# olegiy/manuscript-ocr

Measured on AMD Instinct MI355X. Metric: manuscript pages/sec end-to-end (EAST+TRBA) at 1/2/4/8 MI355X; CER vs CPU ref, higher is better.
Workload: dtype f32 (bf16x3 split operands on the 1x1 / Winograd-domain GEMMs, f32 accumulate)

## Files before the change

### include/msocr.h

```cpp
#ifndef MSOCR_H
#define MSOCR_H
#include <stdint.h>

#ifdef __cplusplus
extern "C" {
#endif

#define MSOCR_F32 0
#define MSOCR_BF16 1

#define MSOCR_OK 0
#define MSOCR_E_ARG (-1)
#define MSOCR_E_LAUNCH (-2)
#define MSOCR_E_NOGPU (-3)

#define MSOCR_CONV_RELU 1u
#define MSOCR_CONV_RESIDUAL 2u
#define MSOCR_CONV_POOL2 4u

typedef struct msocr_conv_desc {
  int32_t dtype;
  int32_t N, H, W, Cin;
  int64_t in_sN, in_sH, in_sW;
  int32_t KH, KW, stride_h, stride_w, pad_h, pad_w;
  int32_t Ho, Wo, Cout;
  int64_t out_ld;
  int64_t res_ld;
  uint32_t flags;
} msocr_conv_desc;

int msocr_conv2d(const msocr_conv_desc* d, const void* in, const void* weight, const float* bias,
                 const void* residual, void* out, void* stream);

#define MSOCR_WINO_2X2 0
#define MSOCR_WINO_4X2 1
#define MSOCR_WINO_4X4 2
int64_t msocr_winograd_workspace_bytes(const msocr_conv_desc* d, int form);
int msocr_winograd_weights_host(int form, const float* w_khwc_host, int Cout, int Cin, float* u_out_host);
int msocr_conv3x3_winograd(const msocr_conv_desc* d, int form, int split, const void* in, const void* u, const float* bias,
                           const void* residual, void* out, void* workspace, void* stream);
int msocr_winograd_input_transform(const msocr_conv_desc* d, int form, const void* in, void* workspace, void* stream);
int msocr_winograd_gemm(const msocr_conv_desc* d, int form, int split, const void* u, void* workspace, void* stream);
int msocr_winograd_output_transform(const msocr_conv_desc* d, int form, const void* workspace, const float* bias, const void* residual,
                                    void* out, void* stream);

int msocr_split_bf16x3_host(const float* w_host, int64_t n, uint16_t* planes_out_host);
int msocr_split_bf16x3_ktile_host(const float* w_host, int64_t nbatch, int64_t rows, int64_t k, uint16_t* planes_out_host);
int msocr_conv1x1_split(const msocr_conv_desc* d, const void* in, const void* weight_planes, const float* bias,
                        const void* residual, void* out, void* stream);
int msocr_conv2d_split(const msocr_conv_desc* d, const void* in, const void* weight_planes, const float* bias,
                       const void* residual, void* out, void* stream);

int64_t msocr_winograd_fused64_workspace_bytes(const msocr_conv_desc* d);
int msocr_conv3x3_winograd_fused64(const msocr_conv_desc* d, int split, const void* in, const void* u, const float* bias,
                                   const void* residual, void* out, void* workspace, void* stream);
int msocr_winograd_fused64_gemm_output(const msocr_conv_desc* d, int split, const void* u, const void* workspace, const float* bias,
                                       const void* residual, void* out, void* stream);

int msocr_normalize_u8(const uint8_t* src, int N, int H, int W, int pad_t, int pad_l, int Hp, int Wp, int cpad,
                       int mode, int dtype, void* out, void* stream);

int msocr_resize_linear_u8(const uint8_t* src, int N, int sh, int sw, uint8_t* dst, int dh, int dw, void* stream);

int msocr_maxpool2d(const void* in, int N, int H, int W, int C, int64_t in_ld, int k, int s, int p, int dtype,
                    void* out, int Ho, int Wo, int64_t out_ld, void* stream);

int msocr_upsample2x_bilinear(const void* in, int N, int H, int W, int C, int64_t in_ld, int dtype, void* out,
// ... 187 lines not shown
```

### manuscript_ocr_amd/_native.py

```python
import ctypes
import os

import torch

_HERE = os.path.dirname(os.path.abspath(__file__))
LIB_PATH = os.path.join(_HERE, "libmsocr.so")

F32, BF16 = 0, 1
CONV_RELU, CONV_RESIDUAL, CONV_POOL2 = 1, 2, 4
WINO_2X2, WINO_4X2, WINO_4X4 = 0, 1, 2

c_i32, c_i64, c_u32 = ctypes.c_int32, ctypes.c_int64, ctypes.c_uint32
c_f32, c_f64, c_vp = ctypes.c_float, ctypes.c_double, ctypes.c_void_p


class ConvDesc(ctypes.Structure):
    _fields_ = [
        ("dtype", c_i32), ("N", c_i32), ("H", c_i32), ("W", c_i32), ("Cin", c_i32),
        ("in_sN", c_i64), ("in_sH", c_i64), ("in_sW", c_i64),
        ("KH", c_i32), ("KW", c_i32), ("stride_h", c_i32), ("stride_w", c_i32), ("pad_h", c_i32), ("pad_w", c_i32),
        ("Ho", c_i32), ("Wo", c_i32), ("Cout", c_i32),
        ("out_ld", c_i64), ("res_ld", c_i64), ("flags", c_u32),
    ]


class JpegInfo(ctypes.Structure):
    _fields_ = [("width", c_i32), ("height", c_i32), ("ncomp", c_i32), ("hs", c_i32 * 3), ("vs", c_i32 * 3),
                ("blocks_w", c_i32 * 3), ("blocks_h", c_i32 * 3), ("supported", c_i32), ("coef_off", c_i64 * 3),
                ("coef_total", c_i64), ("quant", (ctypes.c_uint16 * 64) * 3)]


class AttnWeights(ctypes.Structure):
    _fields_ = [(n, c_vp) for n in ("h2h_wt", "h2h_b", "score_w", "wih_ctx_t", "wih_tok", "whh_t", "b_gates", "gen_wt", "gen_b")]


class AttnSplitWeights(ctypes.Structure):
    _fields_ = [(n, c_vp) for n in ("h2h_p", "whh_p", "gen_p")]


_SIGS = {
    "msocr_conv2d": (c_i32, [ctypes.POINTER(ConvDesc), c_vp, c_vp, c_vp, c_vp, c_vp, c_vp]),
    "msocr_winograd_workspace_bytes": (c_i64, [ctypes.POINTER(ConvDesc), c_i32]),
    "msocr_winograd_weights_host": (c_i32, [c_i32, c_vp, c_i32, c_i32, c_vp]),
    "msocr_conv3x3_winograd": (c_i32, [ctypes.POINTER(ConvDesc), c_i32, c_i32, c_vp, c_vp, c_vp, c_vp, c_vp, c_vp, c_vp]),
    "msocr_winograd_input_transform": (c_i32, [ctypes.POINTER(ConvDesc), c_i32, c_vp, c_vp, c_vp]),
    "msocr_winograd_gemm": (c_i32, [ctypes.POINTER(ConvDesc), c_i32, c_i32, c_vp, c_vp, c_vp]),
    "msocr_winograd_output_transform": (c_i32, [ctypes.POINTER(ConvDesc), c_i32, c_vp, c_vp, c_vp, c_vp, c_vp]),
    "msocr_winograd_fused64_workspace_bytes": (c_i64, [ctypes.POINTER(ConvDesc)]),
    "msocr_conv3x3_winograd_fused64": (c_i32, [ctypes.POINTER(ConvDesc), c_i32, c_vp, c_vp, c_vp, c_vp, c_vp, c_vp, c_vp]),
    "msocr_winograd_fused64_gemm_output": (c_i32, [ctypes.POINTER(ConvDesc), c_i32, c_vp, c_vp, c_vp, c_vp, c_vp, c_vp]),
    "msocr_split_bf16x3_host": (c_i32, [c_vp, c_i64, c_vp]),
    "msocr_split_bf16x3_ktile_host": (c_i32, [c_vp, c_i64, c_i64, c_i64, c_vp]),
    "msocr_conv1x1_split": (c_i32, [ctypes.POINTER(ConvDesc), c_vp, c_vp, c_vp, c_vp, c_vp, c_vp]),
    "msocr_conv2d_split": (c_i32, [ctypes.POINTER(ConvDesc), c_vp, c_vp, c_vp, c_vp, c_vp, c_vp]),
    "msocr_normalize_u8": (c_i32, [c_vp, c_i32, c_i32, c_i32, c_i32, c_i32, c_i32, c_i32, c_i32, c_i32, c_i32, c_vp, c_vp]),
    "msocr_resize_linear_u8": (c_i32, [c_vp, c_i32, c_i32, c_i32, c_vp, c_i32, c_i32, c_vp]),
    "msocr_maxpool2d": (c_i32, [c_vp, c_i32, c_i32, c_i32, c_i32, c_i64, c_i32, c_i32, c_i32, c_i32, c_vp, c_i32, c_i32, c_i64, c_vp]),
    "msocr_upsample2x_bilinear": (c_i32, [c_vp, c_i32, c_i32, c_i32, c_i32, c_i64, c_i32, c_vp, c_i64, c_vp]),
    "msocr_east_head": (c_i32, [c_vp, c_i64, c_i64, c_i32, c_vp, c_vp, c_vp, c_vp, c_vp]),
    "msocr_east_decode": (c_i32, [c_vp, c_vp, c_i32, c_i32, c_i32, c_f32, c_f32, c_i32, c_vp, c_vp, c_i32, c_vp]),
    "msocr_lanms_workspace_bytes": (c_i64, [c_i32, c_i32]),
    "msocr_east_lanms": (c_i32, [c_vp, c_vp, c_i32, c_i32, c_f64, c_vp, c_vp, c_vp, c_vp]),
    "msocr_se_residual": (c_i32, [c_vp, c_vp, c_i32, c_i32, c_i32, c_i32, c_vp, c_vp, c_vp, c_vp, c_vp]),
    "msocr_mean_over_h": (c_i32, [c_vp, c_i32, c_i32, c_i32, c_i32, c_i32, c_vp, c_vp]),
    "msocr_bilstm_recurrent": (c_i32, [c_vp, c_vp, c_i32, c_i32, c_i32, c_vp, c_vp]),
    "msocr_bilstm_recurrent_split": (c_i32, [c_vp, c_vp, c_i32, c_i32, c_i32, c_vp, c_vp]),
    "msocr_attn_greedy": (c_i32, [c_vp, c_vp, ctypes.POINTER(AttnWeights), c_i32, c_i32, c_i32, c_i32, c_i32, c_i32, c_i32, c_i32,
                                  c_vp, c_vp, c_vp]),
    "msocr_attn_greedy_hoisted": (c_i32, [c_vp, c_vp, c_vp, ctypes.POINTER(AttnWeights), ctypes.POINTER(AttnSplitWeights), c_i32, c_i32,
                                          c_i32, c_i32, c_i32, c_i32, c_i32, c_i32, c_vp, c_vp, c_vp]),
# ... 105 lines not shown
```

### manuscript_ocr_amd/csrc/winograd.hip

```cpp
#include <hip/hip_runtime.h>
#include <stdint.h>

#include "conv_common.h"

template <int M> __device__ void wino_bt1(const f32x4 d[M + 2], f32x4 r[M + 2]);
template <int M> __device__ void wino_at1(const f32x4 m[M + 2], f32x4 y[M]);

template <> __device__ __forceinline__ void wino_bt1<2>(const f32x4 d[4], f32x4 r[4]) {
  r[0] = d[0] - d[2];
  r[1] = d[1] + d[2];
  r[2] = d[2] - d[1];
  r[3] = d[1] - d[3];
}
template <> __device__ __forceinline__ void wino_at1<2>(const f32x4 m[4], f32x4 y[2]) {
  y[0] = (m[0] + m[1]) + m[2];
  y[1] = (m[1] - m[2]) - m[3];
}

__device__ __forceinline__ void wino44_bt(const f32x4 d[6], f32x4 r[6]) {
  constexpr float k97_36 = 97.0f / 36.0f, k4_9 = 4.0f / 9.0f, k9_4 = 2.25f, k3_2 = 1.5f, k2_3 = 2.0f / 3.0f;
#pragma unroll
  for (int e = 0; e < 4; ++e) {
    r[0][e] = fmaf(-k97_36, d[2][e], d[0][e]) + d[4][e];
    r[5][e] = fmaf(-k97_36, d[3][e], d[1][e]) + d[5][e];
    const float e1 = fmaf(-k4_9, d[2][e], d[4][e]), o1 = fmaf(k3_2, d[3][e], -k2_3 * d[1][e]);
    const float e2 = fmaf(-k9_4, d[2][e], d[4][e]), o2 = fmaf(k2_3, d[3][e], -k3_2 * d[1][e]);
    r[1][e] = e1 + o1; r[2][e] = e1 - o1;
    r[3][e] = e2 + o2; r[4][e] = e2 - o2;
  }
}
__device__ __forceinline__ void wino44_at(const f32x4 m[6], f32x4 y[4]) {
  constexpr float k3_2 = 1.5f, k2_3 = 2.0f / 3.0f, k9_4 = 2.25f, k4_9 = 4.0f / 9.0f, k27_8 = 3.375f, k8_27 = 8.0f / 27.0f;
#pragma unroll
  for (int e = 0; e < 4; ++e) {
    const float p12 = m[1][e] + m[2][e], d12 = m[1][e] - m[2][e], p34 = m[3][e] + m[4][e], d34 = m[3][e] - m[4][e];
    y[0][e] = (m[0][e] + p12) + p34;
    y[1][e] = fmaf(k3_2, d12, k2_3 * d34);
    y[2][e] = fmaf(k9_4, p12, k4_9 * p34);
    y[3][e] = fmaf(k27_8, d12, k8_27 * d34) + m[5][e];
  }
}
template <> __device__ __forceinline__ void wino_bt1<4>(const f32x4 d[6], f32x4 r[6]) { wino44_bt(d, r); }
template <> __device__ __forceinline__ void wino_at1<4>(const f32x4 m[6], f32x4 y[4]) { wino44_at(m, y); }


struct WinoGeom {
  int N, H, W;
  int TH, TW;
  long Mt;
};

template <int MH, int MW>
__device__ __forceinline__ void wino_input_body(const float* in, long sN, long sH, long sW, int C, WinoGeom g, float* V) {
  constexpr int PH = MH + 2, PW = MW + 2;
  constexpr bool w_first = MH == 4;
  const int cch = C >> 2;
  const long gid = (long)blockIdx.x * 256 + threadIdx.x;
  const long t = gid / cch;
  const int c = (int)(gid - t * cch) << 2;
  if (t >= g.Mt) return;
  const int tw = (int)(t % g.TW);
  const long r = t / g.TW;
  const int th = (int)(r % g.TH);
  const int n = (int)(r / g.TH);
  const int h0 = MH * th - 1, w0 = MW * tw - 1;
  const float* base = in + (long)n * sN + c;
  f32x4 q[PH][PW];
#pragma unroll
  for (int i = 0; i < PH; ++i) {
    const int hi = h0 + i;
    const bool okh = (unsigned)hi < (unsigned)g.H;
    f32x4 d[PW];
#pragma unroll
    for (int j = 0; j < PW; ++j) {
      const int wi = w0 + j;
      const bool ok = okh && (unsigned)wi < (unsigned)g.W;
      const f32x4 v = *reinterpret_cast<const f32x4*>(ok ? base + (long)hi * sH + (long)wi * sW : base);
      d[j] = ok ? v : (f32x4){0.f, 0.f, 0.f, 0.f};
    }
    if constexpr (w_first) {
      wino_bt1<MW>(d, q[i]);
    } else {
#pragma unroll
      for (int j = 0; j < PW; ++j) q[i][j] = d[j];
    }
  }
  const long plane = g.Mt * (long)C;
  float* o = V + t * (long)C + c;
// ... 7 lines not shown
#pragma unroll
      for (int i = 0; i < PH; ++i) *reinterpret_cast<f32x4*>(o + (i * PW + j) * plane) = v[i];
    }
  } else {
#pragma unroll
    for (int i = 0; i < PH; ++i) {
      f32x4 row[PW], v[PW];
#pragma unroll
      for (int j = 0; j < PW; ++j) {
        f32x4 col[PH], hv[PH];
#pragma unroll
        for (int k = 0; k < PH; ++k) col[k] = q[k][j];
        wino_bt1<MH>(col, hv);
        row[j] = hv[i];
      }
      wino_bt1<MW>(row, v);
#pragma unroll
      for (int j = 0; j < PW; ++j) *reinterpret_cast<f32x4*>(o + (i * PW + j) * plane) = v[j];
    }
  }
}

template <int MH, int MW>
__device__ __forceinline__ void wino_output_body(const float* Mw, int Cout, WinoGeom g, const float* bias, const float* res, long res_ld,
                                                 int relu, float* out, long out_ld) {
  constexpr int PH = MH + 2, PW = MW + 2;
  const int cch = Cout >> 2;
  const long gid = (long)blockIdx.x * 256 + threadIdx.x;
  const long t = gid / cch;
  const int c = (int)(gid - t * cch) << 2;
  if (t >= g.Mt) return;
  const int tw = (int)(t % g.TW);
  const long r = t / g.TW;
  const int th = (int)(r % g.TH);
  const int n = (int)(r / g.TH);
  const long plane = g.Mt * (long)Cout;
  const float* mp = Mw + t * (long)Cout + c;
  f32x4 mt[PH][PW];
  if constexpr (MH == 2) {
#pragma unroll
    for (int i = 0; i < PH; ++i)
#pragma unroll
      for (int j = 0; j < PW; ++j) mt[i][j] = *reinterpret_cast<const f32x4*>(mp + (i * PW + j) * plane);
  }
  f32x4 s[MH][PW];
#pragma unroll
  for (int j = 0; j < PW; ++j) {
    f32x4 m[PH], y[MH];
#pragma unroll
    for (int i = 0; i < PH; ++i) m[i] = MH == 2 ? mt[i][j] : *reinterpret_cast<const f32x4*>(mp + (i * PW + j) * plane);
    wino_at1<MH>(m, y);
#pragma unroll
    for (int a = 0; a < MH; ++a) s[a][j] = y[a];
  }
  f32x4 b = {0.f, 0.f, 0.f, 0.f};
  if (bias) b = *reinterpret_cast<const f32x4*>(bias + c);
#pragma unroll
  for (int a = 0; a < MH; ++a) {
    const int ho = MH * th + a;
    if (ho >= g.H) continue;
    f32x4 y[MW];
    wino_at1<MW>(s[a], y);
#pragma unroll
    for (int j = 0; j < MW; ++j) {
      const int wo = MW * tw + j;
      if (wo >= g.W) continue;
      const long pix = ((long)n * g.H + ho) * g.W + wo;
      f32x4 v = y[j] + b;
      if (res) v += *reinterpret_cast<const f32x4*>(res + pix * res_ld + c);
      if (relu) {
        v[0] = fmaxf(v[0], 0.f); v[1] = fmaxf(v[1], 0.f); v[2] = fmaxf(v[2], 0.f); v[3] = fmaxf(v[3], 0.f);
      }
      *reinterpret_cast<f32x4*>(out + pix * out_ld + c) = v;
    }
  }
}

#define WINO_TRANSFORM_KERNELS(PREFIX, MH, MW)                                                                                    \
  __global__ __launch_bounds__(256) void PREFIX##_input_kernel(const float* __restrict__ in, long sN, long sH, long sW, int C,   \
                                                               WinoGeom g, float* __restrict__ V) {                            \
    wino_input_body<MH, MW>(in, sN, sH, sW, C, g, V);                                                                            \
  }                                                                                                                              \
  __global__ __launch_bounds__(256) void PREFIX##_output_kernel(const float* __restrict__ Mw, int Cout, WinoGeom g,              \
                                                                const float* __restrict__ bias, const float* __restrict__ res,  \
                                                                long res_ld, int relu, float* __restrict__ out, long out_ld) {  \
    wino_output_body<MH, MW>(Mw, Cout, g, bias, res, res_ld, relu, out, out_ld);                                                 \
  }
WINO_TRANSFORM_KERNELS(wino, 2, 2)
WINO_TRANSFORM_KERNELS(wino42, 4, 2)
WINO_TRANSFORM_KERNELS(wino44, 4, 4)
#undef WINO_TRANSFORM_KERNELS

static const int kWinoTile[3][2] = {{2, 2}, {4, 2}, {4, 4}};

static int wino_points(int form) { return (kWinoTile[form][0] + 2) * (kWinoTile[form][1] + 2); }

static bool wino_geom(const msocr_conv_desc* d, int form, WinoGeom* g) {
  if (form < MSOCR_WINO_2X2 || form > MSOCR_WINO_4X4 || !d || d->dtype != MSOCR_F32) return false;
  if (d->KH != 3 || d->KW != 3 || d->stride_h != 1 || d->stride_w != 1 || d->pad_h != 1 || d->pad_w != 1) return false;
  if (d->N <= 0 || d->H <= 0 || d->W <= 0 || d->Ho != d->H || d->Wo != d->W) return false;
  if (d->Cin <= 0 || d->Cin % 16 || d->Cout <= 0 || d->Cout % 32) return false;
  if ((long)d->N * ((d->H + 1) / 2) * ((d->W + 1) / 2) > 0x7fffffffL) return false;
  const int mh = kWinoTile[form][0], mw = kWinoTile[form][1];
  g->N = d->N; g->H = d->H; g->W = d->W;
  g->TH = (d->H + mh - 1) / mh; g->TW = (d->W + mw - 1) / mw;
  g->Mt = (long)d->N * g->TH * g->TW;
  return wino_points(form) * g->Mt * (long)(d->Cin > d->Cout ? d->Cin : d->Cout) <= 0x3fffffffffffL;
}

static bool wino_strides_ok(const msocr_conv_desc* d) { return !(d->in_sN % 4 || d->in_sH % 4 || d->in_sW % 4); }

static int wino_check(const msocr_conv_desc* d, int form, WinoGeom* g) {
  if (!wino_geom(d, form, g) || !wino_strides_ok(d) || d->out_ld % 4 || d->out_ld < d->Cout) return MSOCR_E_ARG;
  return MSOCR_OK;
}

static bool wino_gemm_ok(int form, int split) {
  if (split != 0 && split != 1) return false;
  return form == MSOCR_WINO_4X2 || (form == MSOCR_WINO_2X2 && !split) || (form == MSOCR_WINO_4X4 && split);
}

extern "C" int64_t msocr_winograd_workspace_bytes(const msocr_conv_desc* d, int form) {
  WinoGeom g;
  if (!wino_geom(d, form, &g)) return -1;
  return wino_points(form) * g.Mt * ((int64_t)d->Cin + d->Cout) * (int64_t)sizeof(float);
}

static int wino_launch_input(const msocr_conv_desc* d, int form, const WinoGeom& g, const void* in, void* workspace, void* stream) {
// ... 37 lines not shown
  if (bias && ((uintptr_t)bias & 15)) return MSOCR_E_ARG;
  const long nb_out = (g.Mt * (d->Cout / 4) + 255) / 256;
  if (nb_out > 0x7fffffffL) return MSOCR_E_ARG;
  const float* Mw = (const float*)workspace + wino_points(form) * g.Mt * (long)d->Cin;
  const float* rp = has_res ? (const float*)residual : nullptr;
  const int relu = (d->flags & MSOCR_CONV_RELU) ? 1 : 0;
  const dim3 grid((unsigned)nb_out), blk(256);
  hipStream_t st = (hipStream_t)stream;
  float* o = (float*)out;
  if (form == MSOCR_WINO_2X2) MSOCR_LAUNCH(wino_output_kernel, grid, blk, 0, st, Mw, d->Cout, g, bias, rp, (long)d->res_ld, relu, o, (long)d->out_ld);
  else if (form == MSOCR_WINO_4X2) MSOCR_LAUNCH(wino42_output_kernel, grid, blk, 0, st, Mw, d->Cout, g, bias, rp, (long)d->res_ld, relu, o, (long)d->out_ld);
  else MSOCR_LAUNCH(wino44_output_kernel, grid, blk, 0, st, Mw, d->Cout, g, bias, rp, (long)d->res_ld, relu, o, (long)d->out_ld);
  return hipGetLastError() == hipSuccess ? MSOCR_OK : MSOCR_E_LAUNCH;
}

extern "C" int msocr_conv3x3_winograd(const msocr_conv_desc* d, int form, int split, const void* in, const void* u, const float* bias,
                                      const void* residual, void* out, void* workspace, void* stream) {
  if (!u || !wino_gemm_ok(form, split)) return MSOCR_E_ARG;
  int rc = msocr_winograd_input_transform(d, form, in, workspace, stream);
  if (rc != MSOCR_OK) return rc;
  rc = msocr_winograd_gemm(d, form, split, u, workspace, stream);
  if (rc != MSOCR_OK) return rc;
  return msocr_winograd_output_transform(d, form, workspace, bias, residual, out, stream);
}

typedef unsigned int u32x4w __attribute__((ext_vector_type(4)));
#ifndef WINO_FUSED_PFD
#define WINO_FUSED_PFD 3
#endif

typedef __bf16 bf16x8w __attribute__((ext_vector_type(8)));
typedef unsigned int u32x2w __attribute__((ext_vector_type(2)));
template <bool POOL, bool SPLIT = false>
__global__ __launch_bounds__(256, 3) void wino42_fused64_kernel(const float* __restrict__ V, const void* __restrict__ Uv, int Cout,
                                                                 WinoGeom g, const float* __restrict__ bias,
                                                                 const float* __restrict__ res, long res_ld, int relu,
                                                                 float* __restrict__ out, long out_ld) {
  constexpr int K = 64, BM = 32, BN = 32, ROWB = K * 4;
  constexpr int ROWS = 128, PLANE = BM * ROWS;
  constexpr int STAGE_BYTES = SPLIT ? 6 * PLANE : (BM + BN) * ROWB;
  __shared__ __attribute__((aligned(16))) unsigned char smem[2][STAGE_BYTES];
  const int tid = threadIdx.x, lane = tid & 63, wave = tid >> 6;
  const int mi = wave >> 1, nj = wave & 1;
  const int r16 = lane & 15, kg = lane >> 4;
  const int nbn = Cout / BN;
  const long bid = xcd_tile<long>(blockIdx.x, gridDim.x);
// ... 370 lines not shown
    else
      MSOCR_LAUNCH((wino42_fused64_v2_kernel<false>), grid2, blk, 0, st, ws, up, d->Cout, g, bias, rp, (long)d->res_ld, relu, (float*)out, (long)d->out_ld);
    return hipGetLastError() == hipSuccess ? MSOCR_OK : MSOCR_E_LAUNCH;
  }
  if (d->flags & MSOCR_CONV_POOL2) {
    if (split) MSOCR_LAUNCH((wino42_fused64_kernel<true, true>), grid, blk, 0, st, ws, u, d->Cout, g, bias, (const float*)nullptr, 0L, relu, (float*)out, (long)d->out_ld);
    else MSOCR_LAUNCH((wino42_fused64_kernel<true, false>), grid, blk, 0, st, ws, u, d->Cout, g, bias, (const float*)nullptr, 0L, relu, (float*)out, (long)d->out_ld);
  } else {
    if (split) MSOCR_LAUNCH((wino42_fused64_kernel<false, true>), grid, blk, 0, st, ws, u, d->Cout, g, bias, rp, (long)d->res_ld, relu, (float*)out, (long)d->out_ld);
    else MSOCR_LAUNCH((wino42_fused64_kernel<false, false>), grid, blk, 0, st, ws, u, d->Cout, g, bias, rp, (long)d->res_ld, relu, (float*)out, (long)d->out_ld);
  }
  return hipGetLastError() == hipSuccess ? MSOCR_OK : MSOCR_E_LAUNCH;
}

extern "C" int msocr_conv3x3_winograd_fused64(const msocr_conv_desc* d, int split, const void* in, const void* u, const float* bias,
                                              const void* residual, void* out, void* workspace, void* stream) {
  WinoGeom g;
  if ((split != 0 && split != 1) || wino_fused64_check(d, &g) != MSOCR_OK || !u) return MSOCR_E_ARG;
  const int rc = wino_launch_input(d, MSOCR_WINO_4X2, g, in, workspace, stream);
  if (rc != MSOCR_OK) return rc;
  return msocr_winograd_fused64_gemm_output(d, split, u, workspace, bias, residual, out, stream);
}

extern "C" int msocr_winograd_weights_host(int form, const float* w_khwc, int Cout, int Cin, float* u_out) {
  if (form < MSOCR_WINO_2X2 || form > MSOCR_WINO_4X4 || !w_khwc || !u_out || Cout <= 0 || Cin <= 0) return MSOCR_E_ARG;
  static const double G4[4][3] = {{1.0, 0.0, 0.0}, {0.5, 0.5, 0.5}, {0.5, -0.5, 0.5}, {0.0, 0.0, 1.0}};
  static const double G6[6][3] = {{1.0, 0.0, 0.0},
                                  {8.0 / 65, 12.0 / 65, 18.0 / 65},     {8.0 / 65, -12.0 / 65, 18.0 / 65},
                                  {-81.0 / 130, -27.0 / 65, -18.0 / 65}, {-81.0 / 130, 27.0 / 65, -18.0 / 65},
                                  {0.0, 0.0, 1.0}};
  const int PH = kWinoTile[form][0] + 2, PW = kWinoTile[form][1] + 2;
  const double(*Gh)[3] = PH == 6 ? G6 : G4;
  const double(*Gw)[3] = PW == 6 ? G6 : G4;
  const long plane = (long)Cout * Cin;
  for (int co = 0; co < Cout; ++co) {
    const float* w = w_khwc + (long)co * 9 * Cin;
    for (int c = 0; c < Cin; ++c) {
      double gw[6][3];
      for (int xi = 0; xi < PH; ++xi)
        for (int kw = 0; kw < 3; ++kw)
          gw[xi][kw] = Gh[xi][0] * w[(0 * 3 + kw) * Cin + c] + Gh[xi][1] * w[(1 * 3 + kw) * Cin + c] + Gh[xi][2] * w[(2 * 3 + kw) * Cin + c];
      for (int xi = 0; xi < PH; ++xi)
        for (int nu = 0; nu < PW; ++nu)
          u_out[(xi * PW + nu) * plane + (long)co * Cin + c] =
              (float)(gw[xi][0] * Gw[nu][0] + gw[xi][1] * Gw[nu][1] + gw[xi][2] * Gw[nu][2]);
    }
  }
  return MSOCR_OK;
}
```

### manuscript_ocr_amd/ops.py

```python
import ctypes
import os
from typing import NamedTuple

import numpy as np
import torch

from . import _native as nat


PROFILE = None


def _prof_begin():
    if PROFILE is None:
        return None
    e0 = torch.cuda.Event(enable_timing=True)
    e0.record()
    return e0


def _prof_end(e0, kind, work, tag=None):
    if e0 is None or PROFILE is None:
        return
    e1 = torch.cuda.Event(enable_timing=True)
# ... 38 lines not shown
    if torch.cuda.is_current_stream_capturing():
        return torch.empty((nbytes,), dtype=torch.uint8, device=device)
    key = (device.index, torch.cuda.current_stream().cuda_stream)
    buf = _WINO_ARENA.get(key)
    if buf is None or buf.numel() < nbytes:
        buf = None
        _WINO_ARENA.pop(key, None)
        buf = torch.empty((nbytes,), dtype=torch.uint8, device=device)
        _WINO_ARENA[key] = buf
    return buf


WINOGRAD_TALL = int(os.environ.get("MSOCR_WINO_TALL", "1"))


def _tall_pays(H):
    return 24 * (-(-H // 4)) < 16 * (-(-H // 2))


WINOGRAD_SQUARE = int(os.environ.get("MSOCR_WINO_SQUARE", "1"))
WINOGRAD_SQUARE_MIN_CIN = int(os.environ.get("MSOCR_WINO_SQUARE_MIN_CIN", "512"))


def _square_pays(W):
    return 36 * (-(-W // 4)) < 24 * (-(-W // 2))


WINO_FORMS = {nat.WINO_2X2: ("winograd", 16, (2, 2)), nat.WINO_4X2: ("winograd42", 24, (4, 2)), nat.WINO_4X4: ("winograd44", 36, (4, 4))}


def _wino_weights(wh, form):
    Cout, _, _, Cin = wh.shape
    u = torch.empty((WINO_FORMS[form][1], Cout, Cin), dtype=torch.float32)
    nat.check(nat.lib().msocr_winograd_weights_host(form, wh.data_ptr(), Cout, Cin, u.data_ptr()), "winograd_weights_host")
    return u


WINOGRAD_FUSED64 = int(os.environ.get("MSOCR_WINO_FUSED64", "1"))


SPLIT_BF16X3 = int(os.environ.get("MSOCR_SPLIT", "1"))


def split_planes(t):
    th = t.detach().float().cpu().contiguous()
    planes = torch.empty((3,) + tuple(th.shape), dtype=torch.int16)
    nat.check(nat.lib().msocr_split_bf16x3_host(th.data_ptr(), th.numel(), planes.data_ptr()), "split_bf16x3_host")
    return planes.view(torch.bfloat16).to(t.device)


def split_planes_ktile(t, nbatch, rows):
    th = t.detach().float().cpu().contiguous()
    k = th.numel() // (nbatch * rows)
    assert k % 32 == 0 and nbatch * rows * k == th.numel()
    planes = torch.empty((3, nbatch, k // 32, rows, 32), dtype=torch.int16)
# ... 24 lines not shown
    return w


def attach_winograd(w, split=None, square=True):
    Cout, KH, KW, Cin = w.shape
    if (WINOGRAD_MIN_CIN and WINOGRAD_FUSED64 and WINOGRAD_TALL and w.dtype == torch.float32 and KH == 3 and KW == 3 and Cin == 64
            and Cin < WINOGRAD_MIN_CIN and Cout % 32 == 0):
        u42 = _wino_weights(w.detach().cpu().contiguous(), nat.WINO_4X2)
        w._msocr_wino42_fused = u42.to(w.device)
        if (SPLIT_BF16X3 if split is None else split) and (Cout % 64 == 0 or Cout >= 128):
            w._msocr_wino42_fused_split = split_planes(u42).to(w.device)
        return w
    if not (WINOGRAD_MIN_CIN and w.dtype == torch.float32 and KH == 3 and KW == 3 and Cin >= WINOGRAD_MIN_CIN and Cin % 16 == 0
            and Cout % 32 == 0):
        return w
    wh = w.detach().cpu().contiguous()
    w._msocr_wino = _wino_weights(wh, nat.WINO_2X2).to(w.device)
    u42 = _wino_weights(wh, nat.WINO_4X2)
    w._msocr_wino42 = u42.to(w.device)
    if (SPLIT_BF16X3 if split is None else split) and Cin % 32 == 0 and Cout % 64 == 0:
        w._msocr_wino42_split = split_planes_ktile(u42, 24, Cout).to(w.device)
        if WINOGRAD_SQUARE and square and Cin >= WINOGRAD_SQUARE_MIN_CIN:
            w._msocr_wino44_split = split_planes_ktile(_wino_weights(wh, nat.WINO_4X4), 36, Cout).to(w.device)
    return w


def _winograd(d, x, w, u, form, split, bias, residual, out, alg, fused=False, pool2=False):
    N, H, W, Cin = x.shape
    Cout = w.shape[0]
    stem, npts, (mh, mw) = WINO_FORMS[form]
    name = stem + ("_fused" if fused else "") + ("_split" if split else "")
    L = nat.lib()
    nbytes = L.msocr_winograd_fused64_workspace_bytes(ctypes.byref(d)) if fused else L.msocr_winograd_workspace_bytes(ctypes.byref(d), form)
    if nbytes < 0:
        raise nat.NativeError(f"{name}: unsupported shape {tuple(x.shape)} * {tuple(w.shape)} pool2={pool2}")
    parts = min(N, -(-nbytes // WINO_WS_LIMIT))
    per = -(-N // parts)
    ws = _wino_workspace(nbytes if parts == 1 else (nbytes // N) * per, x.device)
    bp = bias.data_ptr() if bias is not None else None
    what = f"msocr_conv3x3_{name} {tuple(x.shape)} * {tuple(w.shape)}"
    TH, TW = -(-H // mh), -(-W // mw)
    out_px = H * W // (4 if pool2 else 1)
    res_io = 2 if residual is not None else 1
    for n0 in range(0, N, per):
        n1 = min(N, n0 + per)
        d.N = n1 - n0
        xp, rp, op = x[n0:n1].data_ptr(), (residual[n0:n1].data_ptr() if residual is not None else None), out[n0:n1].data_ptr()
        if PROFILE is None:
            if fused:
                rc = L.msocr_conv3x3_winograd_fused64(ctypes.byref(d), int(split), xp, u.data_ptr(), bp, rp, op, ws.data_ptr(), _stream())
            else:
                rc = L.msocr_conv3x3_winograd(ctypes.byref(d), form, int(split), xp, u.data_ptr(), bp, rp, op, ws.data_ptr(), _stream())
            nat.check(rc, what)
            continue
        nn, mt = n1 - n0, (n1 - n0) * TH * TW
        e = _prof_begin()
        nat.check(L.msocr_winograd_input_transform(ctypes.byref(d), form, xp, ws.data_ptr(), _stream()), what)
        _prof_end(e, "wino_in", 4.0 * (nn * H * W * Cin + npts * mt * Cin), (mt, Cin))
        e = _prof_begin()
        if fused:
            rc = L.msocr_winograd_fused64_gemm_output(ctypes.byref(d), int(split), u.data_ptr(), ws.data_ptr(), bp, rp, op, _stream())
        else:
            rc = L.msocr_winograd_gemm(ctypes.byref(d), form, int(split), u.data_ptr(), ws.data_ptr(), _stream())
        nat.check(rc, what)
        io = x.element_size() * (nn * H * W * Cin + nn * out_px * Cout * res_io + Cout * 9 * Cin)
        _prof_end(e, "conv_gemm", (alg * nn / N, 2.0 * npts * mt * Cin * Cout, io), (nn * H * W, Cout, 9 * Cin, name))
        if not fused:
            e = _prof_begin()
            nat.check(L.msocr_winograd_output_transform(ctypes.byref(d), form, ws.data_ptr(), bp, rp, op, _stream()), what)
            _prof_end(e, "wino_out", 4.0 * (npts * mt * Cout + nn * H * W * Cout * res_io), (mt, Cout))
    d.N = N


def conv2d(x, w, bias, stride=(1, 1), pad=(0, 0), relu=False, residual=None, out=None, out_hw=None, alg_k=None, pool2=False):
    _need_cuda(x, w, bias, residual, out)
    N, H, W, Cin = x.shape
    Cout, KH, KW, Cw = w.shape
    assert Cw == Cin and w.is_contiguous() and w.dtype == x.dtype and x.stride(3) == 1
# ... 15 lines not shown
    d.dtype = _dt(x)
    d.N, d.H, d.W, d.Cin = N, H, W, Cin
    d.in_sN, d.in_sH, d.in_sW = x.stride(0), x.stride(1), x.stride(2)
    d.KH, d.KW, d.stride_h, d.stride_w, d.pad_h, d.pad_w = KH, KW, sh, sw, ph, pw
    d.Ho, d.Wo, d.Cout = Ho, Wo, Cout
    d.out_ld = _pixel_dense_ld(out)
    flags = (nat.CONV_RELU if relu else 0) | (nat.CONV_POOL2 if pool2 else 0)
    rp = None
    if residual is not None:
        assert residual.shape == out.shape and residual.dtype == x.dtype
        d.res_ld = _pixel_dense_ld(residual)
        flags |= nat.CONV_RESIDUAL
        rp = residual.data_ptr()
    d.flags = flags
    if bias is not None:
        assert bias.dtype == torch.float32 and bias.numel() == Cout and bias.is_contiguous()
    bp = bias.data_ptr() if bias is not None else None
    alg = 2.0 * N * Ho * Wo * Cout * (alg_k if alg_k else KH * KW * Cin)
    if fused:
        up = getattr(w, "_msocr_wino42_fused_split", None) if SPLIT_BF16X3 else None
        u = w._msocr_wino42_fused if up is None else up
        _winograd(d, x, w, u, nat.WINO_4X2, up is not None, bias, residual, out, alg, fused=True, pool2=pool2)
    elif use_wino:
        form, split = nat.WINO_2X2, False
        if WINOGRAD_TALL and _tall_pays(H) and getattr(w, "_msocr_wino42", None) is not None:
            form, u = nat.WINO_4X2, w._msocr_wino42
            up = getattr(w, "_msocr_wino42_split", None)
            if up is not None and SPLIT_BF16X3:
                u, split = up, True
            up44 = getattr(w, "_msocr_wino44_split", None)
            if up44 is not None and SPLIT_BF16X3 and WINOGRAD_SQUARE and _square_pays(W):
                form, u, split = nat.WINO_4X4, up44, True
        _winograd(d, x, w, u, form, split, bias, residual, out, alg)
    else:
        wp = getattr(w, "_msocr_split", None)
        if (wp is None and SPLIT_BF16X3 and not getattr(w, "_msocr_nosplit", False) and _split_eligible(w)
                and not torch.cuda.is_current_stream_capturing()):
            wp = w._msocr_split = split_planes_ktile(w, 1, Cout)
        split = wp is not None and SPLIT_BF16X3 and KH * KW * Cin >= SPLIT_MIN_K and all(v % 4 == 0 for v in x.stride()[:3])
        lean = (split and (KH, KW, sh, sw, ph, pw) == (1, 1, 1, 1, 0, 0) and (Ho, Wo) == (H, W)
                and (H == 1 or x.stride(1) == W * x.stride(2)) and (N == 1 or x.stride(0) == H * W * x.stride(2)))
        e = _prof_begin()
        if split:
            fn = nat.lib().msocr_conv1x1_split if lean else nat.lib().msocr_conv2d_split
            rc = fn(ctypes.byref(d), x.data_ptr(), wp.data_ptr(), bp, rp, out.data_ptr(), _stream())
            nat.check(rc, f"msocr_conv{'1x1' if lean else '2d'}_split {tuple(x.shape)} * {tuple(w.shape)}")
        else:
            rc = nat.lib().msocr_conv2d(ctypes.byref(d), x.data_ptr(), w.data_ptr(), bp, rp, out.data_ptr(), _stream())
            nat.check(rc, f"msocr_conv2d {tuple(x.shape)} * {tuple(w.shape)}")
        io = x.element_size() * (N * H * W * Cin + N * Ho * Wo * Cout * (2 if residual is not None else 1) + Cout * KH * KW * Cin)
        _prof_end(e, "conv_gemm", (alg, 2.0 * N * Ho * Wo * Cout * KH * KW * Cin, io),
                  (N * Ho * Wo, Cout, KH * KW * Cin, "direct_split" if split else "direct"))
    return out


def normalize_u8(imgs_u8, pad_t, pad_l, Hp, Wp, mode, dtype, cpad=4):
# ... 313 lines not shown
```

Before: 79.79.

## Add F(4x4) Winograd with F(4x1) column tail for widths of form 4k+1

For 3x3 convs whose width is 4k+1, the change splits tiles into a 4x4 Winograd main region plus a single-column 4x1 tail (18 transform points) instead of padding a whole extra 4x4 tile column. It adds combined input and output transform kernels, tail weight transforms, and two batched split-bf16 GEMMs, and updates the square-pays heuristic to account for the cheaper tail. The aim is to cut wasted GEMM work on padded columns, which may also make 4x4 eligible for more layers. In exchange it adds an extra GEMM launch and more workspace complexity.

```diff
diff --git a/include/msocr.h b/include/msocr.h
--- a/include/msocr.h
+++ b/include/msocr.h
@@ -43,6 +43,15 @@
 int msocr_winograd_gemm(const msocr_conv_desc* d, int form, int split, const void* u, void* workspace, void* stream);
 int msocr_winograd_output_transform(const msocr_conv_desc* d, int form, const void* workspace, const float* bias, const void* residual,
                                     void* out, void* stream);
+
+int64_t msocr_winograd_coltail_workspace_bytes(const msocr_conv_desc* d);
+int msocr_winograd_coltail_weights_host(const float* w_khwc_host, int Cout, int Cin, float* u_out_host);
+int msocr_conv3x3_winograd_coltail(const msocr_conv_desc* d, const void* in, const void* u44, const void* u41, const float* bias,
+                                   const void* residual, void* out, void* workspace, void* stream);
+int msocr_winograd_coltail_input_transform(const msocr_conv_desc* d, const void* in, void* workspace, void* stream);
+int msocr_winograd_coltail_gemm(const msocr_conv_desc* d, const void* u44, const void* u41, void* workspace, void* stream);
+int msocr_winograd_coltail_output_transform(const msocr_conv_desc* d, const void* workspace, const float* bias, const void* residual,
+                                            void* out, void* stream);
 
 int msocr_split_bf16x3_host(const float* w_host, int64_t n, uint16_t* planes_out_host);
 int msocr_split_bf16x3_ktile_host(const float* w_host, int64_t nbatch, int64_t rows, int64_t k, uint16_t* planes_out_host);
diff --git a/manuscript_ocr_amd/_native.py b/manuscript_ocr_amd/_native.py
--- a/manuscript_ocr_amd/_native.py
+++ b/manuscript_ocr_amd/_native.py
@@ -46,6 +46,12 @@
     "msocr_winograd_input_transform": (c_i32, [ctypes.POINTER(ConvDesc), c_i32, c_vp, c_vp, c_vp]),
     "msocr_winograd_gemm": (c_i32, [ctypes.POINTER(ConvDesc), c_i32, c_i32, c_vp, c_vp, c_vp]),
     "msocr_winograd_output_transform": (c_i32, [ctypes.POINTER(ConvDesc), c_i32, c_vp, c_vp, c_vp, c_vp, c_vp]),
+    "msocr_winograd_coltail_workspace_bytes": (c_i64, [ctypes.POINTER(ConvDesc)]),
+    "msocr_winograd_coltail_weights_host": (c_i32, [c_vp, c_i32, c_i32, c_vp]),
+    "msocr_conv3x3_winograd_coltail": (c_i32, [ctypes.POINTER(ConvDesc), c_vp, c_vp, c_vp, c_vp, c_vp, c_vp, c_vp, c_vp]),
+    "msocr_winograd_coltail_input_transform": (c_i32, [ctypes.POINTER(ConvDesc), c_vp, c_vp, c_vp]),
+    "msocr_winograd_coltail_gemm": (c_i32, [ctypes.POINTER(ConvDesc), c_vp, c_vp, c_vp, c_vp]),
+    "msocr_winograd_coltail_output_transform": (c_i32, [ctypes.POINTER(ConvDesc), c_vp, c_vp, c_vp, c_vp, c_vp]),
     "msocr_winograd_fused64_workspace_bytes": (c_i64, [ctypes.POINTER(ConvDesc)]),
     "msocr_conv3x3_winograd_fused64": (c_i32, [ctypes.POINTER(ConvDesc), c_i32, c_vp, c_vp, c_vp, c_vp, c_vp, c_vp, c_vp]),
     "msocr_winograd_fused64_gemm_output": (c_i32, [ctypes.POINTER(ConvDesc), c_i32, c_vp, c_vp, c_vp, c_vp, c_vp, c_vp]),
diff --git a/manuscript_ocr_amd/csrc/winograd.hip b/manuscript_ocr_amd/csrc/winograd.hip
--- a/manuscript_ocr_amd/csrc/winograd.hip
+++ b/manuscript_ocr_amd/csrc/winograd.hip
@@ -43,27 +43,29 @@
 template <> __device__ __forceinline__ void wino_bt1<4>(const f32x4 d[6], f32x4 r[6]) { wino44_bt(d, r); }
 template <> __device__ __forceinline__ void wino_at1<4>(const f32x4 m[6], f32x4 y[4]) { wino44_at(m, y); }
 
+template <> __device__ __forceinline__ void wino_bt1<1>(const f32x4 d[3], f32x4 r[3]) {
+  r[0] = d[0]; r[1] = d[1]; r[2] = d[2];
+}
+template <> __device__ __forceinline__ void wino_at1<1>(const f32x4 m[3], f32x4 y[1]) { y[0] = (m[0] + m[1]) + m[2]; }
+
 
 struct WinoGeom {
   int N, H, W;
   int TH, TW;
+  int w0;
   long Mt;
 };
 
 template <int MH, int MW>
-__device__ __forceinline__ void wino_input_body(const float* in, long sN, long sH, long sW, int C, WinoGeom g, float* V) {
+__device__ __forceinline__ void wino_input_body(const float* in, long sN, long sH, long sW, int C, const WinoGeom& g, float* V, long t, int c) {
   constexpr int PH = MH + 2, PW = MW + 2;
   constexpr bool w_first = MH == 4;
-  const int cch = C >> 2;
-  const long gid = (long)blockIdx.x * 256 + threadIdx.x;
-  const long t = gid / cch;
-  const int c = (int)(gid - t * cch) << 2;
   if (t >= g.Mt) return;
   const int tw = (int)(t % g.TW);
   const long r = t / g.TW;
   const int th = (int)(r % g.TH);
   const int n = (int)(r / g.TH);
-  const int h0 = MH * th - 1, w0 = MW * tw - 1;
+  const int h0 = MH * th - 1, w0 = g.w0 + MW * tw - 1;
   const float* base = in + (long)n * sN + c;
   f32x4 q[PH][PW];
 #pragma unroll
@@ -117,13 +119,9 @@
 }
 
 template <int MH, int MW>
-__device__ __forceinline__ void wino_output_body(const float* Mw, int Cout, WinoGeom g, const float* bias, const float* res, long res_ld,
-                                                 int relu, float* out, long out_ld) {
+__device__ __forceinline__ void wino_output_body(const float* Mw, int Cout, const WinoGeom& g, const float* bias, const float* res, long res_ld,
+                                                 int relu, float* out, long out_ld, long t, int c) {
   constexpr int PH = MH + 2, PW = MW + 2;
-  const int cch = Cout >> 2;
-  const long gid = (long)blockIdx.x * 256 + threadIdx.x;
-  const long t = gid / cch;
-  const int c = (int)(gid - t * cch) << 2;
   if (t >= g.Mt) return;
   const int tw = (int)(t % g.TW);
   const long r = t / g.TW;
@@ -158,7 +156,7 @@
     wino_at1<MW>(s[a], y);
 #pragma unroll
     for (int j = 0; j < MW; ++j) {
-      const int wo = MW * tw + j;
+      const int wo = g.w0 + MW * tw + j;
       if (wo >= g.W) continue;
       const long pix = ((long)n * g.H + ho) * g.W + wo;
       f32x4 v = y[j] + b;
@@ -171,20 +169,50 @@
   }
 }
 
+__device__ __forceinline__ long wino_thread_tile(int C, int* c) {
+  const int cch = C >> 2;
+  const long gid = (long)blockIdx.x * 256 + threadIdx.x;
+  const long t = gid / cch;
+  *c = (int)(gid - t * cch) << 2;
+  return t;
+}
+
 #define WINO_TRANSFORM_KERNELS(PREFIX, MH, MW)                                                                                    \
   __global__ __launch_bounds__(256) void PREFIX##_input_kernel(const float* __restrict__ in, long sN, long sH, long sW, int C,   \
                                                                WinoGeom g, float* __restrict__ V) {                            \
-    wino_input_body<MH, MW>(in, sN, sH, sW, C, g, V);                                                                            \
+    int c;                                                                                                                       \
+    const long t = wino_thread_tile(C, &c);                                                                                      \
+    wino_input_body<MH, MW>(in, sN, sH, sW, C, g, V, t, c);                                                                      \
   }                                                                                                                              \
   __global__ __launch_bounds__(256) void PREFIX##_output_kernel(const float* __restrict__ Mw, int Cout, WinoGeom g,              \
                                                                 const float* __restrict__ bias, const float* __restrict__ res,  \
                                                                 long res_ld, int relu, float* __restrict__ out, long out_ld) {  \
-    wino_output_body<MH, MW>(Mw, Cout, g, bias, res, res_ld, relu, out, out_ld);                                                 \
+    int c;                                                                                                                       \
+    const long t = wino_thread_tile(Cout, &c);                                                                                   \
+    wino_output_body<MH, MW>(Mw, Cout, g, bias, res, res_ld, relu, out, out_ld, t, c);                                           \
   }
 WINO_TRANSFORM_KERNELS(wino, 2, 2)
 WINO_TRANSFORM_KERNELS(wino42, 4, 2)
 WINO_TRANSFORM_KERNELS(wino44, 4, 4)
 #undef WINO_TRANSFORM_KERNELS
+
+__global__ __launch_bounds__(256) void wino44_input_kernel_coltail(const float* __restrict__ in, long sN, long sH, long sW, int C,
+                                                                   WinoGeom g44, WinoGeom g41, float* __restrict__ V44,
+                                                                   float* __restrict__ V41) {
+  int c;
+  const long t = wino_thread_tile(C, &c);
+  if (t < g44.Mt) wino_input_body<4, 4>(in, sN, sH, sW, C, g44, V44, t, c);
+  else wino_input_body<4, 1>(in, sN, sH, sW, C, g41, V41, t - g44.Mt, c);
+}
+__global__ __launch_bounds__(256) void wino44_output_kernel_coltail(const float* __restrict__ Mw44, const float* __restrict__ Mw41,
+                                                                    int Cout, WinoGeom g44, WinoGeom g41,
+                                                                    const float* __restrict__ bias, const float* __restrict__ res,
+                                                                    long res_ld, int relu, float* __restrict__ out, long out_ld) {
+  int c;
+  const long t = wino_thread_tile(Cout, &c);
+  if (t < g44.Mt) wino_output_body<4, 4>(Mw44, Cout, g44, bias, res, res_ld, relu, out, out_ld, t, c);
+  else wino_output_body<4, 1>(Mw41, Cout, g41, bias, res, res_ld, relu, out, out_ld, t - g44.Mt, c);
+}
 
 static const int kWinoTile[3][2] = {{2, 2}, {4, 2}, {4, 4}};
 
@@ -199,6 +227,7 @@
   const int mh = kWinoTile[form][0], mw = kWinoTile[form][1];
   g->N = d->N; g->H = d->H; g->W = d->W;
   g->TH = (d->H + mh - 1) / mh; g->TW = (d->W + mw - 1) / mw;
+  g->w0 = 0;
   g->Mt = (long)d->N * g->TH * g->TW;
   return wino_points(form) * g->Mt * (long)(d->Cin > d->Cout ? d->Cin : d->Cout) <= 0x3fffffffffffL;
 }
@@ -282,6 +311,85 @@
   rc = msocr_winograd_gemm(d, form, split, u, workspace, stream);
   if (rc != MSOCR_OK) return rc;
   return msocr_winograd_output_transform(d, form, workspace, bias, residual, out, stream);
+}
+
+struct WinoColtail {
+  WinoGeom g44, g41;
+  long v44, mw44, v41, mw41, total;
+};
+
+static bool wino_coltail_geom(const msocr_conv_desc* d, WinoColtail* ct) {
+  WinoGeom g;
+  if (!wino_geom(d, MSOCR_WINO_4X4, &g) || d->W < 5 || d->W % 4 != 1) return false;
+  if (d->Cin % 32 || d->Cout % 64) return false;
+  ct->g44 = g; ct->g44.TW = d->W / 4; ct->g44.Mt = (long)d->N * g.TH * ct->g44.TW;
+  ct->g41 = g; ct->g41.TW = 1; ct->g41.w0 = d->W - 1; ct->g41.Mt = (long)d->N * g.TH;
+  ct->v44 = 0;
+  ct->mw44 = ct->v44 + 36 * ct->g44.Mt * d->Cin;
+  ct->v41 = ct->mw44 + 36 * ct->g44.Mt * d->Cout;
+  ct->mw41 = ct->v41 + 18 * ct->g41.Mt * d->Cin;
+  ct->total = ct->mw41 + 18 * ct->g41.Mt * d->Cout;
+  return true;
+}
+
+static int wino_coltail_check(const msocr_conv_desc* d, WinoColtail* ct) {
+  if (!wino_coltail_geom(d, ct) || !wino_strides_ok(d) || d->out_ld % 4 || d->out_ld < d->Cout) return MSOCR_E_ARG;
+  return MSOCR_OK;
+}
+
+extern "C" int64_t msocr_winograd_coltail_workspace_bytes(const msocr_conv_desc* d) {
+  WinoColtail ct;
+  if (!wino_coltail_geom(d, &ct)) return -1;
+  return ct.total * (int64_t)sizeof(float);
+}
+
+extern "C" int msocr_winograd_coltail_input_transform(const msocr_conv_desc* d, const void* in, void* workspace, void* stream) {
+  WinoColtail ct;
+  if (wino_coltail_check(d, &ct) != MSOCR_OK) return MSOCR_E_ARG;
+  if (!in || !workspace || (((uintptr_t)in | (uintptr_t)workspace) & 15)) return MSOCR_E_ARG;
+  const long nb_in = ((ct.g44.Mt + ct.g41.Mt) * (d->Cin / 4) + 255) / 256;
+  if (nb_in > 0x7fffffffL) return MSOCR_E_ARG;
+  float* ws = (float*)workspace;
+  MSOCR_LAUNCH(wino44_input_kernel_coltail, dim3((unsigned)nb_in), dim3(256), 0, (hipStream_t)stream, (const float*)in, (long)d->in_sN,
+               (long)d->in_sH, (long)d->in_sW, d->Cin, ct.g44, ct.g41, ws + ct.v44, ws + ct.v41);
+  return hipGetLastError() == hipSuccess ? MSOCR_OK : MSOCR_E_LAUNCH;
+}
+
+extern "C" int msocr_winograd_coltail_gemm(const msocr_conv_desc* d, const void* u44, const void* u41, void* workspace, void* stream) {
+  WinoColtail ct;
+  if (wino_coltail_check(d, &ct) != MSOCR_OK || !u44 || !u41 || !workspace) return MSOCR_E_ARG;
+  float* ws = (float*)workspace;
+  const int rc = msocr_internal_gemm_split_batched(ws + ct.v44, (const uint16_t*)u44, ws + ct.mw44, ct.g44.Mt, d->Cout, d->Cin, 36, (hipStream_t)stream);
+  if (rc != MSOCR_OK) return rc;
+  return msocr_internal_gemm_split_batched(ws + ct.v41, (const uint16_t*)u41, ws + ct.mw41, ct.g41.Mt, d->Cout, d->Cin, 18, (hipStream_t)stream);
+}
+
+extern "C" int msocr_winograd_coltail_output_transform(const msocr_conv_desc* d, const void* workspace, const float* bias, const void* residual,
+                                                       void* out, void* stream) {
+  WinoColtail ct;
+  if (wino_coltail_check(d, &ct) != MSOCR_OK || !out || !workspace) return MSOCR_E_ARG;
+  if (((uintptr_t)out | (uintptr_t)workspace) & 15) return MSOCR_E_ARG;
+  const bool has_res = (d->flags & MSOCR_CONV_RESIDUAL) != 0;
+  if (has_res && (!residual || d->res_ld % 4 || d->res_ld < d->Cout || ((uintptr_t)residual & 15))) return MSOCR_E_ARG;
+  if (bias && ((uintptr_t)bias & 15)) return MSOCR_E_ARG;
+  const long nb_out = ((ct.g44.Mt + ct.g41.Mt) * (d->Cout / 4) + 255) / 256;
+  if (nb_out > 0x7fffffffL) return MSOCR_E_ARG;
+  const float* ws = (const float*)workspace;
+  const float* rp = has_res ? (const float*)residual : nullptr;
+  const int relu = (d->flags & MSOCR_CONV_RELU) ? 1 : 0;
+  MSOCR_LAUNCH(wino44_output_kernel_coltail, dim3((unsigned)nb_out), dim3(256), 0, (hipStream_t)stream, ws + ct.mw44, ws + ct.mw41, d->Cout,
+               ct.g44, ct.g41, bias, rp, (long)d->res_ld, relu, (float*)out, (long)d->out_ld);
+  return hipGetLastError() == hipSuccess ? MSOCR_OK : MSOCR_E_LAUNCH;
+}
+
+extern "C" int msocr_conv3x3_winograd_coltail(const msocr_conv_desc* d, const void* in, const void* u44, const void* u41, const float* bias,
+                                              const void* residual, void* out, void* workspace, void* stream) {
+  if (!u44 || !u41) return MSOCR_E_ARG;
+  int rc = msocr_winograd_coltail_input_transform(d, in, workspace, stream);
+  if (rc != MSOCR_OK) return rc;
+  rc = msocr_winograd_coltail_gemm(d, u44, u41, workspace, stream);
+  if (rc != MSOCR_OK) return rc;
+  return msocr_winograd_coltail_output_transform(d, workspace, bias, residual, out, stream);
 }
 
 typedef unsigned int u32x4w __attribute__((ext_vector_type(4)));
@@ -698,13 +806,15 @@
   return msocr_winograd_fused64_gemm_output(d, split, u, workspace, bias, residual, out, stream);
 }
 
+static const double kWinoG6[6][3] = {{1.0, 0.0, 0.0},
+                                     {8.0 / 65, 12.0 / 65, 18.0 / 65},     {8.0 / 65, -12.0 / 65, 18.0 / 65},
+                                     {-81.0 / 130, -27.0 / 65, -18.0 / 65}, {-81.0 / 130, 27.0 / 65, -18.0 / 65},
+                                     {0.0, 0.0, 1.0}};
+
 extern "C" int msocr_winograd_weights_host(int form, const float* w_khwc, int Cout, int Cin, float* u_out) {
   if (form < MSOCR_WINO_2X2 || form > MSOCR_WINO_4X4 || !w_khwc || !u_out || Cout <= 0 || Cin <= 0) return MSOCR_E_ARG;
   static const double G4[4][3] = {{1.0, 0.0, 0.0}, {0.5, 0.5, 0.5}, {0.5, -0.5, 0.5}, {0.0, 0.0, 1.0}};
-  static const double G6[6][3] = {{1.0, 0.0, 0.0},
-                                  {8.0 / 65, 12.0 / 65, 18.0 / 65},     {8.0 / 65, -12.0 / 65, 18.0 / 65},
-                                  {-81.0 / 130, -27.0 / 65, -18.0 / 65}, {-81.0 / 130, 27.0 / 65, -18.0 / 65},
-                                  {0.0, 0.0, 1.0}};
+  const double(*G6)[3] = kWinoG6;
   const int PH = kWinoTile[form][0] + 2, PW = kWinoTile[form][1] + 2;
   const double(*Gh)[3] = PH == 6 ? G6 : G4;
   const double(*Gw)[3] = PW == 6 ? G6 : G4;
@@ -724,3 +834,18 @@
   }
   return MSOCR_OK;
 }
+
+extern "C" int msocr_winograd_coltail_weights_host(const float* w_khwc, int Cout, int Cin, float* u_out) {
+  if (!w_khwc || !u_out || Cout <= 0 || Cin <= 0) return MSOCR_E_ARG;
+  const long plane = (long)Cout * Cin;
+  for (int co = 0; co < Cout; ++co) {
+    const float* w = w_khwc + (long)co * 9 * Cin;
+    for (int c = 0; c < Cin; ++c)
+      for (int xi = 0; xi < 6; ++xi)
+        for (int kw = 0; kw < 3; ++kw)
+          u_out[(xi * 3 + kw) * plane + (long)co * Cin + c] =
+              (float)(kWinoG6[xi][0] * w[(0 * 3 + kw) * Cin + c] + kWinoG6[xi][1] * w[(1 * 3 + kw) * Cin + c] +
+                      kWinoG6[xi][2] * w[(2 * 3 + kw) * Cin + c]);
+  }
+  return MSOCR_OK;
+}
diff --git a/manuscript_ocr_amd/ops.py b/manuscript_ocr_amd/ops.py
--- a/manuscript_ocr_amd/ops.py
+++ b/manuscript_ocr_amd/ops.py
@@ -84,8 +84,16 @@
 WINOGRAD_SQUARE_MIN_CIN = int(os.environ.get("MSOCR_WINO_SQUARE_MIN_CIN", "512"))
 
 
+WINOGRAD_COLTAIL = int(os.environ.get("MSOCR_WINO_COLTAIL", "1"))
+
+
+def _coltail(W):
+    return bool(WINOGRAD_COLTAIL) and W % 4 == 1 and W >= 5
+
+
 def _square_pays(W):
-    return 36 * (-(-W // 4)) < 24 * (-(-W // 2))
+    points = 36 * (W // 4) + 18 if _coltail(W) else 36 * (-(-W // 4))
+    return points < 24 * (-(-W // 2))
 
 
 WINO_FORMS = {nat.WINO_2X2: ("winograd", 16, (2, 2)), nat.WINO_4X2: ("winograd42", 24, (4, 2)), nat.WINO_4X4: ("winograd44", 36, (4, 4))}
@@ -93,6 +101,10 @@
 
 def _wino_weights(wh, form):
     Cout, _, _, Cin = wh.shape
+    if form == "coltail":
+        u = torch.empty((18, Cout, Cin), dtype=torch.float32)
+        nat.check(nat.lib().msocr_winograd_coltail_weights_host(wh.data_ptr(), Cout, Cin, u.data_ptr()), "winograd_coltail_weights_host")
+        return u
     u = torch.empty((WINO_FORMS[form][1], Cout, Cin), dtype=torch.float32)
     nat.check(nat.lib().msocr_winograd_weights_host(form, wh.data_ptr(), Cout, Cin, u.data_ptr()), "winograd_weights_host")
     return u
@@ -163,16 +175,20 @@
         w._msocr_wino42_split = split_planes_ktile(u42, 24, Cout).to(w.device)
         if WINOGRAD_SQUARE and square and Cin >= WINOGRAD_SQUARE_MIN_CIN:
             w._msocr_wino44_split = split_planes_ktile(_wino_weights(wh, nat.WINO_4X4), 36, Cout).to(w.device)
+            w._msocr_wino41_split = split_planes_ktile(_wino_weights(wh, "coltail"), 18, Cout).to(w.device)
     return w
 
 
-def _winograd(d, x, w, u, form, split, bias, residual, out, alg, fused=False, pool2=False):
+def _winograd(d, x, w, u, form, split, bias, residual, out, alg, fused=False, pool2=False, u41=None):
     N, H, W, Cin = x.shape
     Cout = w.shape[0]
     stem, npts, (mh, mw) = WINO_FORMS[form]
     name = stem + ("_fused" if fused else "") + ("_split" if split else "")
     L = nat.lib()
-    nbytes = L.msocr_winograd_fused64_workspace_bytes(ctypes.byref(d)) if fused else L.msocr_winograd_workspace_bytes(ctypes.byref(d), form)
+    if u41 is not None:
+        nbytes = L.msocr_winograd_coltail_workspace_bytes(ctypes.byref(d))
+    else:
+        nbytes = L.msocr_winograd_fused64_workspace_bytes(ctypes.byref(d)) if fused else L.msocr_winograd_workspace_bytes(ctypes.byref(d), form)
     if nbytes < 0:
         raise nat.NativeError(f"{name}: unsupported shape {tuple(x.shape)} * {tuple(w.shape)} pool2={pool2}")
     parts = min(N, -(-nbytes // WINO_WS_LIMIT))
@@ -188,13 +204,29 @@
         d.N = n1 - n0
         xp, rp, op = x[n0:n1].data_ptr(), (residual[n0:n1].data_ptr() if residual is not None else None), out[n0:n1].data_ptr()
         if PROFILE is None:
-            if fused:
+            if u41 is not None:
+                rc = L.msocr_conv3x3_winograd_coltail(ctypes.byref(d), xp, u.data_ptr(), u41.data_ptr(), bp, rp, op, ws.data_ptr(), _stream())
+            elif fused:
                 rc = L.msocr_conv3x3_winograd_fused64(ctypes.byref(d), int(split), xp, u.data_ptr(), bp, rp, op, ws.data_ptr(), _stream())
             else:
                 rc = L.msocr_conv3x3_winograd(ctypes.byref(d), form, int(split), xp, u.data_ptr(), bp, rp, op, ws.data_ptr(), _stream())
             nat.check(rc, what)
             continue
         nn, mt = n1 - n0, (n1 - n0) * TH * TW
+        if u41 is not None:
+            mt44, mt41 = nn * TH * (W // 4), nn * TH
+            rows, mt = 36 * mt44 + 18 * mt41, mt44 + mt41
+            e = _prof_begin()
+            nat.check(L.msocr_winograd_coltail_input_transform(ctypes.byref(d), xp, ws.data_ptr(), _stream()), what)
+            _prof_end(e, "wino_in", 4.0 * (nn * H * W * Cin + rows * Cin), (mt, Cin))
+            e = _prof_begin()
+            nat.check(L.msocr_winograd_coltail_gemm(ctypes.byref(d), u.data_ptr(), u41.data_ptr(), ws.data_ptr(), _stream()), what)
+            io = x.element_size() * (nn * H * W * Cin + nn * out_px * Cout * res_io + Cout * 9 * Cin)
+            _prof_end(e, "conv_gemm", (alg * nn / N, 2.0 * rows * Cin * Cout, io), (nn * H * W, Cout, 9 * Cin, name))
+            e = _prof_begin()
+            nat.check(L.msocr_winograd_coltail_output_transform(ctypes.byref(d), ws.data_ptr(), bp, rp, op, _stream()), what)
+            _prof_end(e, "wino_out", 4.0 * (rows * Cout + nn * H * W * Cout * res_io), (mt, Cout))
+            continue
         e = _prof_begin()
         nat.check(L.msocr_winograd_input_transform(ctypes.byref(d), form, xp, ws.data_ptr(), _stream()), what)
         _prof_end(e, "wino_in", 4.0 * (nn * H * W * Cin + npts * mt * Cin), (mt, Cin))
@@ -256,7 +288,7 @@
         u = w._msocr_wino42_fused if up is None else up
         _winograd(d, x, w, u, nat.WINO_4X2, up is not None, bias, residual, out, alg, fused=True, pool2=pool2)
     elif use_wino:
-        form, split = nat.WINO_2X2, False
+        form, split, u41 = nat.WINO_2X2, False, None
         if WINOGRAD_TALL and _tall_pays(H) and getattr(w, "_msocr_wino42", None) is not None:
             form, u = nat.WINO_4X2, w._msocr_wino42
             up = getattr(w, "_msocr_wino42_split", None)
@@ -265,7 +297,8 @@
             up44 = getattr(w, "_msocr_wino44_split", None)
             if up44 is not None and SPLIT_BF16X3 and WINOGRAD_SQUARE and _square_pays(W):
                 form, u, split = nat.WINO_4X4, up44, True
-        _winograd(d, x, w, u, form, split, bias, residual, out, alg)
+                u41 = getattr(w, "_msocr_wino41_split", None) if _coltail(W) else None
+        _winograd(d, x, w, u, form, split, bias, residual, out, alg, u41=u41)
     else:
         wp = getattr(w, "_msocr_split", None)
         if (wp is None and SPLIT_BF16X3 and not getattr(w, "_msocr_nosplit", False) and _split_eligible(w)
```

Result: faster. 82.87 (median of 6 runs) (+3.9%).
